# JulHoltzDevelopers/WavesAndEigenvalues.jl

Hardware: AMD Instinct MI355X
Metric: eigenpairs/sec (higher is better)
Workload: dtype f64

## Files before the change

### include/waehip.h

```cpp
#ifndef WAEHIP_H
#define WAEHIP_H
#include <stdint.h>

#ifdef __cplusplus
extern "C" {
#endif

typedef struct wae_family wae_family;

#define WAE_OK                 0
#define WAE_WARN_MAXITER       1
#define WAE_WARN_STAGNATION    2
#define WAE_ERR_INVALID       -1
#define WAE_ERR_BREAKDOWN     -2
#define WAE_ERR_EIGS          -3
#define WAE_ERR_NAN           -4
#define WAE_ERR_HIP           -5

#define WAE_OP_N 0
#define WAE_OP_T 1
#define WAE_OP_C 2

#define WAE_CSC 0
#define WAE_CSR 1
// ... 197 lines not shown
int wae_bench_triad(int32_t device, int64_t n, int32_t reps, double *gbs_out);

int wae_debug_spmv(wae_family *h, int32_t which, int32_t level, int32_t mode, const double *coeffs, int32_t ncoef, const double *X,
                   const double *B, double *Y, double *B2, int32_t r, int32_t op, double jac_w, const uint8_t *cmask, int32_t flags,
                   int64_t *n_in_q, int64_t *n_out_q);

int wae_debug_prolong(wae_family *h, int32_t level, const double *X, const double *B, double *Y, double *norms, int32_t r, const uint8_t *cmask,
                      int32_t flags);

int wae_debug_vcycle(wae_family *h, int32_t level, const double *coeffs, int32_t ncoef, const double *B, double *Y, int32_t r, int32_t op,
                     int32_t flags, const uint8_t *cmask);

enum {
    WAE_VEC_DOTS = 0, WAE_VEC_NORMS, WAE_VEC_DOTS_MULTI, WAE_VEC_AXPY_NEG, WAE_VEC_LINCOMB, WAE_VEC_LINCOMB_ADD, WAE_VEC_AXPY_NEG_NORM,
    WAE_VEC_AXPY_NEG_MULTI, WAE_VEC_DOTS2, WAE_VEC_AXPY2, WAE_VEC_LINCOMB_REP, WAE_VEC_SCALE_INV, WAE_VEC_MASK_COLS, WAE_VEC_EXTRACT_COLS,
    WAE_VEC_BEYN_ACCUM, WAE_VEC_PT_GEMM_BATCH, WAE_VEC_PT_AXPBY_COLS, WAE_VEC_PT_PROJECT, WAE_VEC_DENSE
};
int wae_debug_vec(int32_t device, int32_t op, const int64_t *sz, int32_t nsz, double *const *bufs, const int64_t *lens, int32_t nbuf,
                  const uint8_t *cmask, const int32_t *perm, int32_t *status_out);

enum { WAE_GMRES_INIT = 0, WAE_GMRES_STEP, WAE_GMRES_PAIR, WAE_GMRES_SOLVE_Y };
int wae_debug_gmres(int32_t device, int32_t nb, int32_t m, int32_t histcap, int64_t n, const double *bnorm, const int64_t *ev,
                    const double *evd, int32_t nev, double *pool, int64_t plen, double *cstate, double *dstate, double *snap_relres,
                    int32_t *snap_int, uint8_t *snap_cmask, double *snap_rescale, double *snap_sv, double *snap_vsq);

#ifdef __cplusplus
}
#endif
#endif
```

### wavesandeigenvalues.jl_amd/_lib.py

```python
from __future__ import annotations

import ctypes as C
import os

import numpy as np

_HERE = os.path.dirname(os.path.abspath(__file__))
LIB_PATH = os.environ.get("WAE_LIB_PATH") or os.path.join(_HERE, "csrc", "libwaehip.so")

WAE_OK, WAE_WARN_MAXITER, WAE_WARN_STAGNATION = 0, 1, 2
WAE_ERR_INVALID, WAE_ERR_BREAKDOWN, WAE_ERR_EIGS, WAE_ERR_NAN, WAE_ERR_HIP = -1, -2, -3, -4, -5
OP_N, OP_T, OP_C = 0, 1, 2
CSC, CSR = 0, 1


class SolveInfo(C.Structure):
    _fields_ = [("iters_max", C.c_int32), ("iters_total", C.c_int32), ("n_unconverged", C.c_int32),
                ("levels", C.c_int32), ("relres_max", C.c_double), ("seconds", C.c_double)]

    def as_dict(self):
        return {k: getattr(self, k) for k, _ in self._fields_}


class WaeError(RuntimeError):
# ... 14 lines not shown
    "wae_p1_assemble_cpoint", "wae_p1_assemble_boundary_cpoint", "wae_p2_assemble_cpoint", "wae_p2_assemble_boundary_cpoint",
    "wae_p1_assemble_source", "wae_p1_assemble_source_cpoint", "wae_p2_assemble_source", "wae_p2_assemble_source_cpoint", "wae_forced_response",
    "wae_p2_shape_sensitivity", "wae_p1_shape_sensitivity_cpoint", "wae_p2_shape_sensitivity_cpoint", "wae_p2_shape_sensitivity_flame",
    "wae_bloch_numbering", "wae_bloch_numbering_info", "wae_bloch_numbering_get", "wae_bloch_numbering_free", "wae_bloch_fold",
    "wae_octosplit", "wae_octosplit_info", "wae_octosplit_get", "wae_octosplit_prolong", "wae_octosplit_free",
    "wae_octosplit_prolongator", "wae_solver_setup_nested",
    "wae_octosplit_p2_info", "wae_octosplit_prolongator_p2", "wae_octosplit_prolong_p2", "wae_p2_embedding",
    "wae_locator_create", "wae_locator_info", "wae_locator_find", "wae_locator_set_p2", "wae_locator_weights", "wae_locator_sample",
    "wae_locator_free",
]
BLOCH_IMAGE, BLOCH_AXIS = 1, 2
TALL_MAXCOLS = 64

(VEC_DOTS, VEC_NORMS, VEC_DOTS_MULTI, VEC_AXPY_NEG, VEC_LINCOMB, VEC_LINCOMB_ADD, VEC_AXPY_NEG_NORM, VEC_AXPY_NEG_MULTI, VEC_DOTS2, VEC_AXPY2,
 VEC_LINCOMB_REP, VEC_SCALE_INV, VEC_MASK_COLS, VEC_EXTRACT_COLS, VEC_BEYN_ACCUM, VEC_PT_GEMM_BATCH, VEC_PT_AXPBY_COLS,
 VEC_PT_PROJECT, VEC_DENSE) = range(19)
GMRES_INIT, GMRES_STEP, GMRES_PAIR, GMRES_SOLVE_Y = range(4)


def lib():
    global _lib
    if _lib is not None:
        return _lib
    if not os.path.exists(LIB_PATH):
        raise ImportError(f"{LIB_PATH} not found: build it with `python -c 'import __graft_entry__ as g; g.build()'` "
                          "(hipcc --offload-arch=gfx950). There is no CPU fallback for the product path.")
    L = C.CDLL(LIB_PATH)
    dp = C.POINTER(C.c_double)
    vpp = C.POINTER(C.c_void_p)
    L.wae_last_error.restype = C.c_char_p
    L.wae_version.restype = C.c_char_p
# ... 248 lines not shown
```

### wavesandeigenvalues.jl_amd/csrc/beyn.hip

```cpp
#include <cmath>

#include "solver.h"

static void small_solve(std::vector<zc> &A, std::vector<zc> &b, int n) {
    std::vector<char> dead(n, 0);
    double amax = 0.0;
    for (const zc &a : A) amax = std::max(amax, std::abs(a));
    for (int k = 0; k < n; ++k) {
        int p = k;
        double best = 0.0;
        for (int i = k; i < n; ++i) { const double v = std::abs(A[(size_t)k * n + i]); if (v > best) { best = v; p = i; } }
        if (!(best > 1e-14 * amax)) { dead[k] = 1; continue; }
        if (p != k) {
            for (int j = 0; j < n; ++j) std::swap(A[(size_t)j * n + k], A[(size_t)j * n + p]);
            std::swap(b[k], b[p]);
        }
        const zc inv = 1.0 / A[(size_t)k * n + k];
        for (int i = k + 1; i < n; ++i) {
            const zc f = A[(size_t)k * n + i] * inv;
            if (f == zc(0)) continue;
            for (int j = k + 1; j < n; ++j) A[(size_t)j * n + i] -= f * A[(size_t)j * n + k];
            b[i] -= f * b[k];
        }
    }
// ... 24 lines not shown
    R.wait_w();
    if (R.W.n < R.kact.size() * (size_t)cap * vecl) {
        const size_t need = R.kact.size() * (size_t)cap * vecl;
        const int dev = h->device;
        RbState *Rp = &R;
        R.w_job = std::async(std::launch::async, [Rp, need, dev]() {
            HIP_CHECK(hipSetDevice(dev));
            Rp->W.alloc(need);
        });
    }
    R.Hk.assign(R.kact.size() * (size_t)cap * cap * l, zc(0));
    R.g.assign((size_t)cap * l, zc(0));
    R.Vi.reserve(vecl);
    HIP_CHECK(hipMemcpyAsync(R.Vi.p, Vinter, vecl * sizeof(cplx), hipMemcpyDeviceToDevice, h->stream));
    R.vi_valid = true;
    R.hb.reserve((size_t)4 * (cap + 4) * l); R.alpha.reserve(l); R.alpha2.reserve((size_t)cap * l);
}

static void rb_append_block(wae_family *h, int cnt, const std::vector<std::vector<std::vector<zc>>> &pck) {
    RbState &R = h->rb;
    hipStream_t st = h->stream;
    const int64_t d = h->d;
    const int l = R.l, cap = R.cap, S = R.S;
    const size_t vecl = (size_t)d * l;
    std::vector<cplx> hh((size_t)(S + cnt) * cnt * l), n0((size_t)cnt * l), n1(l);
    const OpDev A0 = h->ops[0].dev(WAE_OP_N);
    cplx *qn = R.Q + (size_t)S * vecl;
    for (int j = 0; j < cnt; ++j) launch_norms(qn + (size_t)j * vecl, d, l, h->partial.p, R.hb.p + (size_t)j * l, st);
    rb_d2h(h, R.hb.p, n0.data(), (size_t)cnt * l);
    static const bool multi_axpy = !(getenv("WAE_RB_MULTI_AXPY") && atoi(getenv("WAE_RB_MULTI_AXPY")) == 0);
    const bool fits = (size_t)S * cnt * l * sizeof(cplx) <= 60 * 1024;
// ... 21 lines not shown
        }
        launch_norms(q, d, l, h->partial.p, R.hb.p, st);
        rb_d2h(h, R.hb.p, n1.data(), l);
        for (int c = 0; c < l; ++c) {
            const double nrm0 = n0[(size_t)j * l + c].x;
            n1[c] = (n1[c].x > 1e-9 * nrm0 && nrm0 > 0.0) ? cplx{n1[c].x, 0.0} : cplx{0.0, 0.0};
        }
        R.alpha.upload(n1.data(), l, st);
        launch_scale_inv(q, R.alpha.p, q, d, l, st);
        HIP_CHECK(hipStreamSynchronize(st));
    }
    launch_dots_multi(qn, vecl, cnt, R.Vi.p, vecl, 1, d, l, h->partial.p, R.hb.p, st);
    rb_d2h(h, R.hb.p, hh.data(), (size_t)cnt * l);
    for (int j = 0; j < cnt; ++j)
        for (int c = 0; c < l; ++c) R.g[(size_t)(S + j) * l + c] = zc(hh[(size_t)j * l + c].x, hh[(size_t)j * l + c].y);
    for (size_t ki = 0; ki < R.kact.size(); ++ki) {
        R.wait_w();
        cplx *Wk = R.W.p + ki * (size_t)cap * vecl;
        cplx *wn = Wk + (size_t)S * vecl;
        upload_pc(h, pck[ki]);
        for (int j = 0; j < cnt; ++j)
            launch_spmv(A0, pc_level(h, 0), l, qn + (size_t)j * vecl, wn + (size_t)j * vecl, nullptr, 0.0, l, MODE_AX, st);
        zc *H = &R.Hk[ki * (size_t)cap * cap * l];
        launch_dots_multi(R.Q, vecl, S + cnt, wn, vecl, cnt, d, l, h->partial.p, R.hb.p, st);
        rb_d2h(h, R.hb.p, hh.data(), (size_t)(S + cnt) * cnt * l);
        for (int i = 0; i < S + cnt; ++i)
            for (int j = 0; j < cnt; ++j)
                for (int c = 0; c < l; ++c) {
                    const cplx v = hh[((size_t)i * cnt + j) * l + c];
                    H[((size_t)(S + j) * cap + i) * l + c] = zc(v.x, v.y);
                }
        zc herm_factor(0);
        bool herm = false;
        {
            static const bool herm_on = !(getenv("WAE_RB_HERMITIAN") && atoi(getenv("WAE_RB_HERMITIAN")) == 0);
            const int kterm = R.kact[ki], pl = h->term_plane[kterm];
            const LevelOp &L0 = h->ops[0];
            for (size_t g = 0; g < L0.groups.size() && herm_on && !herm; ++g)
                for (int q = 0; q < L0.groups[g].nplanes; ++q)
                    if (h->slot_plane[0][(size_t)L0.groups[g].plane0 + q] == pl && L0.groups[g].symmetric && L0.groups[g].is_real) {
// ... 208 lines not shown
            const bool guess = p.guess && R.S > 0;
            const double ta = now_s();
            if (guess) {
                std::vector<cplx> Y;
                if (next_Y.valid()) {
                    Y = next_Y.get();
                    if (p0 + spc < npts) next_Y = launch_coeffs(p0 + spc);
                } else {
                    Y = rb_guess_coeffs(h, p.coeff_table + (size_t)p0 * 2 * T, ns);
                }
                rb_apply_guess(h, Y, ns, h->Xs.p);
            }
            const double tb = now_s();
            h->vc_light = guess && p.light_cycle;
            const int its = solve_chunk(h, bt, pcs, h->Bs.p, h->Xs.p, p.tol, p.maxit, &ci.li, nullptr, guess);
            launch_beyn_accum(h->Xs.p, bt.nb, d, lg, ns, h->zw_dev.p, h->zw_dev.p + ns, npow, Ad, st, p.l_total, p.col0 + cg, h->perm());
            if (rbdbg) HIP_CHECK(hipStreamSynchronize(st));
            const double tc = now_s();
            if (p.keep == BeynPass::raw_to_store) {
                for (int s = 0; s < ns; ++s)
                    launch_extract_cols(h->Xs.p, bt.nb, s * l, l, Q + (size_t)(p.slot0 + p0 + s) * vecl, d, st);
            } else if (p.keep == BeynPass::into_basis || (its > p.enrich_its && R.S + ns <= R.cap)) {
                for (int s = 0; s < ns; ++s)
                    launch_extract_cols(h->Xs.p, bt.nb, s * l, l, Q + (size_t)(R.S + s) * vecl, d, st);
                rb_append(h, ns);
            }
            if (rbdbg) {
                HIP_CHECK(hipStreamSynchronize(st));
                t_guess += tb - ta; t_solve += tc - tb; t_append += now_s() - tc;
            }
        }
// ... 78 lines not shown
```

### wavesandeigenvalues.jl_amd/csrc/debug.hip

```cpp
#include <algorithm>
#include <vector>

#include "solver.h"

namespace {
struct StreamGuard {
    hipStream_t s = nullptr;
    ~StreamGuard() { if (s) (void)hipStreamDestroy(s); }
};
int64_t span(int64_t nv, int64_t stride, int64_t blk) { return nv > 0 ? (nv - 1) * stride + blk : 0; }
void fill_xorshift(std::vector<cplx> &hx) {
    uint64_t s = 0x9E3779B97F4A7C15ull;
    for (auto &v : hx) { s ^= s << 13; s ^= s >> 7; s ^= s << 17; v.x = (double)(s & 0xFFFFF) / 524288.0 - 1.0; v.y = (double)((s >> 20) & 0xFFFFF) / 524288.0 - 1.0; }
}
template <class F> double mean_ms(hipStream_t st, int reps, F &&one) {
    for (int i = 0; i < 3; ++i) one();
    hipEvent_t e0, e1;
    HIP_CHECK(hipEventCreate(&e0));
    HIP_CHECK(hipEventCreate(&e1));
    HIP_CHECK(hipEventRecord(e0, st));
    for (int i = 0; i < reps; ++i) one();
    HIP_CHECK(hipEventRecord(e1, st));
    HIP_CHECK(hipEventSynchronize(e1));
    float ms = 0.f;
// ... 47 lines not shown
            cplx *out = need(2, (int64_t)nv * nb);
            if (scale) launch_dots_scaled(V, (size_t)stride, nv, W, n, (int)nb, want_partial(), out, scale, st, mask());
            else launch_dots(V, (size_t)stride, nv, W, n, (int)nb, want_partial(), out, st, mask());
            break;
        }
        case WAE_VEC_NORMS:
            launch_norms(need(0, blk), n, (int)nb, want_partial(), need(1, nb), st, mask());
            break;
        case WAE_VEC_DOTS_MULTI: {
            const int nv = count_of(2), nw = count_of(3);
            WAE_REQUIRE(nw >= 1 && nw <= 4, "nw in 1..4");
            const cplx *V = need(0, span(nv, S(4), blk)), *W = need(1, span(nw, S(5), blk));
            launch_dots_multi(V, (size_t)S(4), nv, W, (size_t)S(5), nw, n, (int)nb, want_partial(), need(2, (int64_t)nv * nw * nb), st);
            break;
        }
        case WAE_VEC_AXPY_NEG: case WAE_VEC_LINCOMB: case WAE_VEC_LINCOMB_ADD: {
            const int nv = count_of(2);
            const cplx *V = need(0, span(nv, S(3), blk)), *c = need(1, (int64_t)nv * nb);
            cplx *W = need(2, blk);
            if (op == WAE_VEC_AXPY_NEG) launch_axpy_neg(V, (size_t)S(3), nv, c, W, n, (int)nb, st, mask());
            else if (op == WAE_VEC_LINCOMB) launch_lincomb(V, (size_t)S(3), nv, c, W, n, (int)nb, st);
            else launch_lincomb_add(V, (size_t)S(3), nv, c, W, n, (int)nb, st);
            break;
        }
        case WAE_VEC_AXPY_NEG_NORM: {
            const int nv = count_of(2);
            const cplx *V = need(0, span(nv, S(3), blk)), *h = need(1, (int64_t)nv * nb), *base = opt(4, blk);
            cplx *W = need(2, blk), *norms = need(3, nb), *inv = opt(5, nb);
            launch_axpy_neg_norm(V, (size_t)S(3), nv, h, W, n, (int)nb, want_partial(), norms, st, mask(), base, inv);
            break;
// ... 27 lines not shown
            launch_lincomb_rep(need(0, span(nv, S(3), n * l)), (size_t)S(3), nv, need(1, (int64_t)nv * nb), need(2, blk), n, (int)nb, (int)l, st);
            break;
        }
        case WAE_VEC_SCALE_INV:
            launch_scale_inv(need(0, blk), need(1, nb), need(2, blk), n, (int)nb, st, mask());
            break;
        case WAE_VEC_MASK_COLS:
            launch_mask_cols(need(0, blk), need(1, nb), n, (int)nb, st);
            break;
        case WAE_VEC_EXTRACT_COLS: {
            const int64_t off = S(2), l = S(3);
            WAE_REQUIRE(l >= 1 && off + l <= nb, "columns off .. off+l-1 must lie inside the batch");
            launch_extract_cols(need(0, blk), (int)nb, (int)off, (int)l, need(1, n * l), n, st);
            break;
        }
        case WAE_VEC_BEYN_ACCUM: {
            const int64_t l = S(2), nsys = S(3), npow = S(4), lA = S(5) > 0 ? S(5) : l, c0 = S(6);
            WAE_REQUIRE(l >= 1 && nsys >= 1 && nsys * l <= nb && npow >= 1 && npow <= 64 && c0 + l <= lA && lA <= 4096, "bad moment shape");
            if (perm) {
                for (int64_t i = 0; i < n; ++i) WAE_REQUIRE(perm[i] >= 0 && perm[i] < n, "perm entry out of range");
                pm.upload(perm, (size_t)n, st);
            }
            launch_beyn_accum(need(0, blk), (int)nb, n, (int)l, (int)nsys, need(1, nsys), need(2, nsys), (int)npow, need(3, npow * lA * n), st,
                              (int)S(5), (int)c0, perm ? pm.p : nullptr);
            break;
        }
        case WAE_VEC_PT_GEMM_BATCH: {
            const int k = count_of(2), T = count_of(4);
            WAE_REQUIRE(k >= 1 && T >= 1, "k >= 1, T >= 1");
            launch_pt_gemm_batch(need(0, span(k, S(3), blk)), (size_t)S(3), k, need(1, (int64_t)k * T * nb), need(2, blk * T), n, T, (int)nb, st);
            break;
        }
        case WAE_VEC_PT_AXPBY_COLS:
            launch_pt_axpby_cols(need(0, 2 * nb), need(1, blk), need(2, blk), need(3, blk), n, (int)nb, st);
            break;
        case WAE_VEC_PT_PROJECT: {
            const int nd = count_of(2);
            WAE_REQUIRE(nd >= 1, "nd >= 1");
            launch_pt_project(need(0, blk), need(1, blk), need(2, (int64_t)nd * nb), nd, n, (int)nb, st);
// ... 443 lines not shown
```

### wavesandeigenvalues.jl_amd/csrc/family.h

```cpp
#pragma once
#include <algorithm>
#include <chrono>
#include <future>

#include "amg.h"
#include "tiles.h"

struct RbState {
    cplx *Q = nullptr;
    int cap = 0, l = 0, S = 0;
    std::vector<int> kact;
    std::vector<zc> Hk;
    std::vector<zc> g;
    DevBuf<cplx> W, Vi, hb, alpha, alpha2, ycoef;
    std::future<void> w_job;
    void wait_w() { if (w_job.valid()) w_job.get(); }
    bool vi_valid = false;
    ~RbState() { if (w_job.valid()) w_job.wait(); }
};

struct wae_family {
    bool vc_light = false;
    int device = 0;
    hipStream_t stream = nullptr;
    int64_t d = 0;
    int T = 0;
    std::vector<int> term_plane;
    std::vector<zc> term_scale;
    std::vector<int64_t> term_nnz;
    int nplanes = 0;
    std::vector<CsrZ> planes0;
    std::vector<int> perm_h;
    DevBuf<int> perm_dev;
    std::vector<int> tile_row_ptr;
    const int *perm() const { return perm_dev.p; }
    std::vector<LevelOp> ops;
    std::vector<std::vector<int>> slot_plane;
    std::vector<Transfer> xfer;
    int64_t nc = 0;
    DevBuf<cplx> dense_planes, Ainv;
    DevBuf<int> dstatus;
    bool solver_ready = false;
    double jac_w = 0.8;
    double jac_w_post = 0.9;
    double jac_w_light = 0.5;
    int nsweeps = 1, restart = 30, NB = 64;
    std::vector<DevBuf<cplx>> lx, lb, lt;
    DevBuf<cplx> V, W, Z, Xs, Bs, U, partial, hdev, ydev, pcdev, one_dev, io_a, io_b, zw_dev;
    DevBuf<cplx> vsq;
    DevBuf<cplx> rbQ;
// ... 73 lines not shown
```

### wavesandeigenvalues.jl_amd/csrc/setup.hip

```cpp
#include <atomic>
#include <cmath>
#include <exception>
#include <limits>
#include <map>
#include <memory>
#include <tuple>

#include "family.h"

OpDev LevelOp::dev(int op) const {
    OpDev o;
    memset(&o, 0, sizeof(o));
    o.ngroups = (int)groups.size();
    o.nplanes_total = nplanes;
    o.n = n;
    o.diag = diag.p;
    o.conj_diag = (op == WAE_OP_C) ? 1 : 0;
    o.tiles = !tiles.ready ? nullptr : (op == WAE_OP_N || tiles.all_symmetric) ? &tiles.dev : (tiles.ready_t ? &tiles.dev_t : nullptr);
    {
        const LongRows &LR = (op == WAE_OP_N) ? long_n : long_t;
        o.nlong = LR.n;
        o.long_rows = LR.rows.p; o.long_ptr = LR.ptr.p; o.long_col = LR.col.p; o.long_slot = LR.slot.p;
        o.long_val = LR.val.p; o.long_acc = LR.acc.p; o.long_part = LR.part.p;
        o.long_conj = (op == WAE_OP_C) ? 1 : 0;
// ... 608 lines not shown
            h->term_plane[k] = (int)h->planes0.size();
            h->term_scale[k] = 1.0;
            h->planes0.push_back(std::move(A));
        }
    }
    h->nplanes = (int)h->planes0.size();
}
static void renumber_fine_level(wae_family *h, const SetupEnv &env) {
    const double tq0 = now_s();
    TilePlan plan = plan_tiles(union_pattern(h->planes0), 256, env.wcap, TILE_THICK);
    const double tq1 = now_s();
    if (!plan.perm.empty()) {
        host_ranges(h->nplanes, h->nplanes, [&](int64_t q, int64_t, int) { h->planes0[q] = permute_symmetric(h->planes0[q], plan.perm, plan.iperm); });
        h->perm_h = plan.perm;
        h->perm_dev.upload(h->perm_h.data(), h->perm_h.size(), h->stream);
        h->tile_row_ptr = plan.row_ptr;
    }
    if (env.debug)
        fprintf(stderr, "[create] tile plan %.3f s (%zu tiles, largest window %d), permutation of the planes %.3f s\n", tq1 - tq0,
                plan.row_ptr.empty() ? (size_t)0 : plan.row_ptr.size() - 1, plan.wmax, now_s() - tq1);
}

extern "C" int wae_family_create(wae_family **out, int64_t d, int32_t T, int32_t index_bytes, int32_t base, int32_t orientation,
                                 const void *const *ptr, const void *const *idx, const double *const *val, int32_t device) {
    return wae_family_create_opts(out, d, T, index_bytes, base, orientation, ptr, idx, val, device, nullptr, 0);
}

extern "C" int wae_family_create_opts(wae_family **out, int64_t d, int32_t T, int32_t index_bytes, int32_t base, int32_t orientation,
                                      const void *const *ptr, const void *const *idx, const double *const *val, int32_t device,
                                      const double *opts, int32_t nopts) {
// ... 491 lines not shown
```

### wavesandeigenvalues.jl_amd/csrc/vec.hip

```cpp
#include <type_traits>

#include "block_reduce.h"
#include "kernel_helpers.h"

__global__ void fill_zero_kernel(cplx *X, size_t count) {
    for (size_t e = (size_t)blockIdx.x * 256 + threadIdx.x; e < count; e += (size_t)gridDim.x * 256) X[e] = cplx{0.0, 0.0};
}
void launch_fill_zero(cplx *X, size_t count, hipStream_t st) {
    if (!count) return;
    hipLaunchKernelGGL(fill_zero_kernel, dim3(grid_for(count)), dim3(256), 0, st, X, count);
    HIP_CHECK(hipGetLastError());
}
void launch_copy(const cplx *X, cplx *Y, size_t count, hipStream_t st) {
    if (!count) return;
    HIP_CHECK(hipMemcpyAsync(Y, X, count * sizeof(cplx), hipMemcpyDeviceToDevice, st));
}
__global__ void add_kernel(const cplx *__restrict__ X, cplx *__restrict__ Y, size_t count) {
    for (size_t e = (size_t)blockIdx.x * 256 + threadIdx.x; e < count; e += (size_t)gridDim.x * 256) {
        cplx a = X[e], b = Y[e];
        Y[e] = cplx{a.x + b.x, a.y + b.y};
    }
}
void launch_add(const cplx *X, cplx *Y, size_t count, hipStream_t st) {
    if (!count) return;
// ... 138 lines not shown
        }
    }
}
void launch_dots_multi(const cplx *V, size_t sv, int nv, const cplx *W, size_t sw, int nw, int64_t n, int nb, cplx *partial, cplx *out,
                       hipStream_t st) {
    if (nb < 1 || nb > 256 || nw < 1 || nw > 4) throw WaeError(WAE_ERR_INVALID, "dots_multi: nb in 1..256, nw in 1..4");
    int done = 0;
    while (done < nv) {
        const int chunk = std::min(8, nv - done);
        const int nblk = 768;
        hipLaunchKernelGGL((dots_multi_kernel<8, 4>), dim3(nblk), dim3(256), 0, st, V + (size_t)done * sv, sv, chunk, W, sw, nw, n, nb, partial);
        HIP_CHECK(hipGetLastError());
        const int count = chunk * nw * nb;
        launch_reduce_partials(partial, nblk, count, out + (size_t)done * nw * nb, 0, st);
        done += chunk;
    }
}
void launch_dots(const cplx *V, size_t stride, int nv, const cplx *W, int64_t n, int nb, cplx *partial, cplx *out, hipStream_t st,
                 const unsigned char *cmask) {
    dots_impl(V, stride, nv, W, n, nb, partial, out, 0, st, cmask);
}
void launch_dots_scaled(const cplx *V, size_t stride, int nv, const cplx *W, int64_t n, int nb, cplx *partial, cplx *out, const cplx *scale,
                        hipStream_t st, const unsigned char *cmask) {
    dots_impl(V, stride, nv, W, n, nb, partial, out, 0, st, cmask, scale);
}
void launch_norms(const cplx *X, int64_t n, int nb, cplx *partial, cplx *out, hipStream_t st, const unsigned char *cmask) {
    dots_impl(X, 0, 1, X, n, nb, partial, out, 1, st, cmask);
}

constexpr int AXU = 8;
// ... 557 lines not shown
        }
        __syncthreads();
    }
}
void launch_beyn_accum(const cplx *Xi, int nb, int64_t d, int l, int nsys, const cplx *w, const cplx *z, int npow, cplx *A, hipStream_t st,
                       int lA, int c0, const int *perm) {
    if (lA <= 0) lA = l;
    if (!d || nb < 1) return;
    if (nb > 256) throw WaeError(WAE_ERR_INVALID, "beyn_accum: nb must be in 1..256");
    int TR = 2048 / (nb + 1);
    if (TR > 32) TR = 32;
    if (TR < 1) TR = 1;
    const int64_t tiles = (d + TR - 1) / TR;
    const unsigned grid = (unsigned)std::min<int64_t>(tiles, 4096);
    hipLaunchKernelGGL(beyn_accum_kernel, dim3(grid), dim3(256), (size_t)TR * (nb + 1) * sizeof(cplx), st, Xi, nb, d, l, nsys, w, z, npow, A, lA, c0, TR, perm);
    HIP_CHECK(hipGetLastError());
}

__global__ __launch_bounds__(256) void gmres_init_kernel(GmresDev S, const cplx *__restrict__ beta, const unsigned char *__restrict__ done, int use_mask) {
    __shared__ int act[256];
    const int b = threadIdx.x;
    int a = 0;
    if (b < S.nb) {
        S.g[b] = cplx{beta[b].x, 0.0};
        S.sv[b] = 1.0;
        S.vsq[b] = cplx{1.0, 0.0};
        S.conv[b] = done[b] ? 1 : 0;
        S.steps[b] = 0;
        a = done[b] ? 0 : 1;
    }
// ... 322 lines not shown
```

### wavesandeigenvalues.jl_amd/csrc/wae_internal.h

```cpp
#pragma once
#include <hip/hip_runtime.h>
#include <algorithm>
#include <cmath>
#include <complex>
#include <cstdint>
#include <cstdio>
#include <cstring>
#include <stdexcept>
#include <string>
#include <vector>

#include "../../include/waehip.h"

typedef std::complex<double> zc;
typedef double2 cplx;

struct WaeError : std::runtime_error {
    int code;
    WaeError(int c, const std::string &m) : std::runtime_error(m), code(c) {}
};
void wae_set_error(const std::string &m);
int wae_internal_device(const wae_family *h);
hipStream_t wae_internal_stream(const wae_family *h);

// ... 262 lines not shown
void launch_lincomb_add(const cplx *V, size_t stride, int nv, const cplx *y, cplx *X, int64_t n, int nb, hipStream_t s);
void launch_norms(const cplx *X, int64_t n, int nb, cplx *partial, cplx *out, hipStream_t s, const unsigned char *cmask = nullptr);
void launch_scale_inv(const cplx *X, const cplx *alpha, cplx *Y, int64_t n, int nb, hipStream_t s, const unsigned char *cmask = nullptr);
void launch_axpby1(cplx a, const cplx *x, cplx b, const cplx *y, cplx *out, size_t n, hipStream_t s, int conj_x = 0);
void launch_add(const cplx *X, cplx *Y, size_t count, hipStream_t s);
void launch_colmajor_to_inter(const cplx *Xc, int64_t d, int r, cplx *Xi, int nb, hipStream_t s, const int *perm = nullptr);
void launch_inter_to_colmajor(const cplx *Xi, int nb, int64_t d, int r, cplx *Xc, hipStream_t s, const int *perm = nullptr);
void launch_replicate(const cplx *Vc, int64_t d, int l, cplx *Xi, int nb, hipStream_t s, const int *perm = nullptr);
constexpr int PROLONG_NORM_BLOCKS = 1024;
void launch_prolong_add(const int *ptr, const int *col, const double *val, int64_t n, const cplx *Xc, const cplx *X, cplx *Y, int nb, hipStream_t s,
                        const unsigned char *cmask = nullptr, cplx *partial = nullptr, cplx *norms = nullptr);
void launch_reduce_partials(const cplx *partial, int nblk, int count, cplx *out, int do_sqrt, hipStream_t s, const cplx *scale = nullptr,
                            cplx *inv_out = nullptr);
void launch_dots_multi(const cplx *V, size_t sv, int nv, const cplx *W, size_t sw, int nw, int64_t n, int nb, cplx *partial, cplx *out,
                       hipStream_t s);
void launch_gather_rows(const cplx *X, const int *rows, int64_t nrows, int nb, cplx *out, hipStream_t s);
void launch_scatter_add_rows(const cplx *D, const int *rows, int64_t nrows, int nb, cplx *X, hipStream_t s);
void launch_extract_cols(const cplx *X, int nb, int off, int l, cplx *out, int64_t n, hipStream_t s);
void launch_lincomb_rep(const cplx *Q, size_t stride, int nv, const cplx *y, cplx *X, int64_t n, int nb, int l, hipStream_t s);
void launch_mask_cols(cplx *X, const cplx *keep, int64_t n, int nb, hipStream_t s);
void launch_beyn_accum(const cplx *Xi, int nb, int64_t d, int l, int nsys, const cplx *w, const cplx *z, int npow, cplx *A, hipStream_t s,
                       int lA = 0, int c0 = 0, const int *perm = nullptr);
void launch_pt_gemm_batch(const cplx *V, size_t stride, int k, const cplx *G, cplx *U, int64_t d, int T, int nb, hipStream_t s);
void launch_pt_spmv_batch(const OpDev &op, const cplx *pc, const int *plane_col, const cplx *U, int nin, cplx *Y, int nb, int accumulate,
                          hipStream_t s);
void launch_pt_axpby_cols(const cplx *coef, const cplx *x, const cplx *y, cplx *out, int64_t d, int nb, hipStream_t s);
void launch_pt_project(cplx *vk, const cplx *v0, const cplx *dots, int nd, int64_t d, int nb, hipStream_t s);
struct GmresDev {
    int nb, m, histcap;
    cplx *R;
    double *cs;
    cplx *sn;
    cplx *g;
    double *sv;
    cplx *vsq;
    int *conv, *steps, *iters, *histlen, *stalled;
    double *relres, *bnorm;
// ... 20 lines not shown
```

Before: 4.359.

## Batch reduced-basis projections across terms and add row-ordered Beyn accumulation

Adds a dots_terms kernel that computes projections of the basis Q against two term blocks per launch, reusing each loaded basis tile for both terms. All term SpMVs are issued first, then one batched projection and a single device-to-host copy replace the per-term dots_multi launches and copies. Adds a beyn_accum_rows kernel that reads X through the inverse permutation and writes the moment matrix A row-contiguously, aiming for coalesced stores instead of scattered ones. Both paths are on by default behind environment toggles; they add new buffers and shared-memory use, and the dots kernel hardcodes 768 blocks of 512 threads.

Result: no change. 4.396 (median of 6 runs) (+0.8%).

```diff
diff --git a/dev/chunk_boundary_stats.py b/dev/chunk_boundary_stats.py
--- /dev/null
+++ b/dev/chunk_boundary_stats.py
@@ -0,0 +1,62 @@
+#!/usr/bin/env python3
+import csv
+import os
+import re
+import sys
+
+ROOT = os.path.dirname(os.path.dirname(os.path.abspath(__file__)))
+PASSES = 4
+D, L, NS, NPOW = 995328, 8, 8, 4
+
+
+def short(name):
+    return re.sub(r"^void ", "", name.split("(")[0])
+
+
+def load(path):
+    out = {}
+    for r in csv.DictReader(open(path)):
+        k = short(r["Name"])
+        c, t = out.get(k, (0, 0.0))
+        out[k] = (c + int(r["Calls"]), t + float(r["TotalDurationNs"]) / 1e6)
+    return out
+
+
+par, chg = load(sys.argv[1]), load(sys.argv[2])
+par2 = load(sys.argv[3]) if len(sys.argv) > 3 else None
+keys = sorted(set(par) | set(chg), key=lambda k: -max(par.get(k, (0, 0))[1], chg.get(k, (0, 0))[1]))
+dst = os.path.join(ROOT, "profiles", "chunk_boundary_kernel_stats.csv")
+with open(dst, "w", newline="") as f:
+    w = csv.writer(f)
+    head = ["kernel", "parent_calls", "parent_total_ms", "parent_ms_per_pass", "change_calls", "change_total_ms", "change_ms_per_pass",
+            "change_minus_parent_ms_per_pass"]
+    if par2:
+        head.append("second_parent_minus_parent_ms_per_pass")
+    w.writerow(head)
+    for k in keys:
+        pc, pt = par.get(k, (0, 0.0))
+        cc, ct = chg.get(k, (0, 0.0))
+        if max(pt, ct) / PASSES < 0.2:
+            continue
+        row = [k, pc, f"{pt:.2f}", f"{pt / PASSES:.2f}", cc, f"{ct:.2f}", f"{ct / PASSES:.2f}", f"{(ct - pt) / PASSES:.2f}"]
+        if par2:
+            row.append(f"{(par2.get(k, (0, 0.0))[1] - pt) / PASSES:.2f}")
+        w.writerow(row)
+    tp, tc = sum(v[1] for v in par.values()), sum(v[1] for v in chg.values())
+    w.writerow(["all kernels", "", f"{tp:.2f}", f"{tp / PASSES:.2f}", "", f"{tc:.2f}", f"{tc / PASSES:.2f}", f"{(tc - tp) / PASSES:.2f}"]
+               + ([f"{(sum(v[1] for v in par2.values()) - tp) / PASSES:.2f}"] if par2 else []))
+print("wrote", dst)
+
+acc_bytes = 16 * D * L * (NS + 2 * NPOW)
+for side, tab in (("parent", par), ("change", chg)):
+    for k in ("beyn_accum_kernel", "beyn_accum_rows_kernel"):
+        if k in tab:
+            c, t = tab[k]
+            us = 1e3 * t / c
+            print(f"{side:7s} {k:26s} {c:5d} launches  {acc_bytes / 1e9:.3f} GB  {us:7.1f} us  {acc_bytes / us / 1e3:7.1f} GB/s")
+    for k, nw in (("dots_multi_kernel<8, 4>", 4), ("dots_terms_kernel<8, 4>", 8)):
+        if k in tab:
+            c, t = tab[k]
+            us = 1e3 * t / c
+            b = 16 * D * L * (8 + nw)
+            print(f"{side:7s} {k:26s} {c:5d} launches  <= {b / 1e9:.3f} GB  {us:7.1f} us  <= {b / us / 1e3:7.1f} GB/s (mean over all launches)")
diff --git a/include/waehip.h b/include/waehip.h
--- a/include/waehip.h
+++ b/include/waehip.h
@@ -235,7 +235,8 @@
 enum {
     WAE_VEC_DOTS = 0, WAE_VEC_NORMS, WAE_VEC_DOTS_MULTI, WAE_VEC_AXPY_NEG, WAE_VEC_LINCOMB, WAE_VEC_LINCOMB_ADD, WAE_VEC_AXPY_NEG_NORM,
     WAE_VEC_AXPY_NEG_MULTI, WAE_VEC_DOTS2, WAE_VEC_AXPY2, WAE_VEC_LINCOMB_REP, WAE_VEC_SCALE_INV, WAE_VEC_MASK_COLS, WAE_VEC_EXTRACT_COLS,
-    WAE_VEC_BEYN_ACCUM, WAE_VEC_PT_GEMM_BATCH, WAE_VEC_PT_AXPBY_COLS, WAE_VEC_PT_PROJECT, WAE_VEC_DENSE
+    WAE_VEC_BEYN_ACCUM, WAE_VEC_PT_GEMM_BATCH, WAE_VEC_PT_AXPBY_COLS, WAE_VEC_PT_PROJECT, WAE_VEC_DENSE,
+    WAE_VEC_BEYN_ACCUM_ROWS, WAE_VEC_DOTS_TERMS
 };
 int wae_debug_vec(int32_t device, int32_t op, const int64_t *sz, int32_t nsz, double *const *bufs, const int64_t *lens, int32_t nbuf,
                   const uint8_t *cmask, const int32_t *perm, int32_t *status_out);
diff --git a/wavesandeigenvalues.jl_amd/_lib.py b/wavesandeigenvalues.jl_amd/_lib.py
--- a/wavesandeigenvalues.jl_amd/_lib.py
+++ b/wavesandeigenvalues.jl_amd/_lib.py
@@ -52,7 +52,7 @@
 
 (VEC_DOTS, VEC_NORMS, VEC_DOTS_MULTI, VEC_AXPY_NEG, VEC_LINCOMB, VEC_LINCOMB_ADD, VEC_AXPY_NEG_NORM, VEC_AXPY_NEG_MULTI, VEC_DOTS2, VEC_AXPY2,
  VEC_LINCOMB_REP, VEC_SCALE_INV, VEC_MASK_COLS, VEC_EXTRACT_COLS, VEC_BEYN_ACCUM, VEC_PT_GEMM_BATCH, VEC_PT_AXPBY_COLS,
- VEC_PT_PROJECT, VEC_DENSE) = range(19)
+ VEC_PT_PROJECT, VEC_DENSE, VEC_BEYN_ACCUM_ROWS, VEC_DOTS_TERMS) = range(21)
 GMRES_INIT, GMRES_STEP, GMRES_PAIR, GMRES_SOLVE_Y = range(4)
 
 
diff --git a/wavesandeigenvalues.jl_amd/csrc/beyn.hip b/wavesandeigenvalues.jl_amd/csrc/beyn.hip
--- a/wavesandeigenvalues.jl_amd/csrc/beyn.hip
+++ b/wavesandeigenvalues.jl_amd/csrc/beyn.hip
@@ -62,7 +62,8 @@
     R.Vi.reserve(vecl);
     HIP_CHECK(hipMemcpyAsync(R.Vi.p, Vinter, vecl * sizeof(cplx), hipMemcpyDeviceToDevice, h->stream));
     R.vi_valid = true;
-    R.hb.reserve((size_t)4 * (cap + 4) * l); R.alpha.reserve(l); R.alpha2.reserve((size_t)cap * l);
+    R.hb.reserve((size_t)4 * (cap + 4) * l * std::max<size_t>(1, R.kact.size())); R.alpha.reserve(l); R.alpha2.reserve((size_t)cap * l);
+    R.tpart.reserve(DOTS_TERMS_PARTIAL * l);
 }
 
 static void rb_append_block(wae_family *h, int cnt, const std::vector<std::vector<std::vector<zc>>> &pck) {
@@ -114,16 +115,36 @@
     rb_d2h(h, R.hb.p, hh.data(), (size_t)cnt * l);
     for (int j = 0; j < cnt; ++j)
         for (int c = 0; c < l; ++c) R.g[(size_t)(S + j) * l + c] = zc(hh[(size_t)j * l + c].x, hh[(size_t)j * l + c].y);
-    for (size_t ki = 0; ki < R.kact.size(); ++ki) {
+    static const bool terms_fused = !(getenv("WAE_RB_TERMS_FUSED") && atoi(getenv("WAE_RB_TERMS_FUSED")) == 0);
+    const size_t nk = R.kact.size(), hcnt = (size_t)(S + cnt) * cnt * l;
+    std::vector<cplx> hall;
+    if (terms_fused && nk > 1) {
+        R.wait_w();
+        for (size_t ki = 0; ki < nk; ++ki) {
+            cplx *wn = R.W.p + ki * (size_t)cap * vecl + (size_t)S * vecl;
+            upload_pc(h, pck[ki]);
+            for (int j = 0; j < cnt; ++j)
+                launch_spmv(A0, pc_level(h, 0), l, qn + (size_t)j * vecl, wn + (size_t)j * vecl, nullptr, 0.0, l, MODE_AX, st);
+        }
+        R.hb.reserve(nk * hcnt); R.tpart.reserve(DOTS_TERMS_PARTIAL * l);
+        launch_dots_terms(R.Q, vecl, S + cnt, R.W.p + (size_t)S * vecl, vecl, (size_t)cap * vecl, (int)nk, cnt, d, l, R.tpart.p, R.hb.p, hcnt, st);
+        hall.resize(nk * hcnt);
+        rb_d2h(h, R.hb.p, hall.data(), nk * hcnt);
+    }
+    for (size_t ki = 0; ki < nk; ++ki) {
         R.wait_w();
         cplx *Wk = R.W.p + ki * (size_t)cap * vecl;
         cplx *wn = Wk + (size_t)S * vecl;
-        upload_pc(h, pck[ki]);
-        for (int j = 0; j < cnt; ++j)
-            launch_spmv(A0, pc_level(h, 0), l, qn + (size_t)j * vecl, wn + (size_t)j * vecl, nullptr, 0.0, l, MODE_AX, st);
         zc *H = &R.Hk[ki * (size_t)cap * cap * l];
-        launch_dots_multi(R.Q, vecl, S + cnt, wn, vecl, cnt, d, l, h->partial.p, R.hb.p, st);
-        rb_d2h(h, R.hb.p, hh.data(), (size_t)(S + cnt) * cnt * l);
+        if (hall.empty()) {
+            upload_pc(h, pck[ki]);
+            for (int j = 0; j < cnt; ++j)
+                launch_spmv(A0, pc_level(h, 0), l, qn + (size_t)j * vecl, wn + (size_t)j * vecl, nullptr, 0.0, l, MODE_AX, st);
+            launch_dots_multi(R.Q, vecl, S + cnt, wn, vecl, cnt, d, l, h->partial.p, R.hb.p, st);
+            rb_d2h(h, R.hb.p, hh.data(), hcnt);
+        } else {
+            std::copy(hall.begin() + ki * hcnt, hall.begin() + (ki + 1) * hcnt, hh.begin());
+        }
         for (int i = 0; i < S + cnt; ++i)
             for (int j = 0; j < cnt; ++j)
                 for (int c = 0; c < l; ++c) {
@@ -362,7 +383,11 @@
             const double tb = now_s();
             h->vc_light = guess && p.light_cycle;
             const int its = solve_chunk(h, bt, pcs, h->Bs.p, h->Xs.p, p.tol, p.maxit, &ci.li, nullptr, guess);
-            launch_beyn_accum(h->Xs.p, bt.nb, d, lg, ns, h->zw_dev.p, h->zw_dev.p + ns, npow, Ad, st, p.l_total, p.col0 + cg, h->perm());
+            static const bool accum_rows = !(getenv("WAE_ACCUM_ROWS") && atoi(getenv("WAE_ACCUM_ROWS")) == 0);
+            if (accum_rows && (!h->perm() || h->iperm()))
+                launch_beyn_accum_rows(h->Xs.p, bt.nb, d, lg, ns, h->zw_dev.p, h->zw_dev.p + ns, npow, Ad, st, p.l_total, p.col0 + cg, h->iperm());
+            else
+                launch_beyn_accum(h->Xs.p, bt.nb, d, lg, ns, h->zw_dev.p, h->zw_dev.p + ns, npow, Ad, st, p.l_total, p.col0 + cg, h->perm());
             if (rbdbg) HIP_CHECK(hipStreamSynchronize(st));
             const double tc = now_s();
             if (p.keep == BeynPass::raw_to_store) {
diff --git a/wavesandeigenvalues.jl_amd/csrc/debug.hip b/wavesandeigenvalues.jl_amd/csrc/debug.hip
--- a/wavesandeigenvalues.jl_amd/csrc/debug.hip
+++ b/wavesandeigenvalues.jl_amd/csrc/debug.hip
@@ -85,6 +85,15 @@
             launch_dots_multi(V, (size_t)S(4), nv, W, (size_t)S(5), nw, n, (int)nb, want_partial(), need(2, (int64_t)nv * nw * nb), st);
             break;
         }
+        case WAE_VEC_DOTS_TERMS: {
+            const int nv = count_of(2), nw = count_of(3), nt = count_of(6);
+            WAE_REQUIRE(nw >= 1 && nw <= 4 && nt >= 1, "nw in 1..4, nt >= 1");
+            const cplx *V = need(0, span(nv, S(4), blk)), *W = need(1, span(nt, S(7), span(nw, S(5), blk)));
+            partial.alloc(DOTS_TERMS_PARTIAL * (size_t)nb);
+            launch_dots_terms(V, (size_t)S(4), nv, W, (size_t)S(5), (size_t)S(7), nt, nw, n, (int)nb, partial.p, need(2, (int64_t)nt * nv * nw * nb),
+                              (size_t)nv * nw * nb, st);
+            break;
+        }
         case WAE_VEC_AXPY_NEG: case WAE_VEC_LINCOMB: case WAE_VEC_LINCOMB_ADD: {
             const int nv = count_of(2);
             const cplx *V = need(0, span(nv, S(3), blk)), *c = need(1, (int64_t)nv * nb);
@@ -142,15 +151,27 @@
             launch_extract_cols(need(0, blk), (int)nb, (int)off, (int)l, need(1, n * l), n, st);
             break;
         }
-        case WAE_VEC_BEYN_ACCUM: {
+        case WAE_VEC_BEYN_ACCUM: case WAE_VEC_BEYN_ACCUM_ROWS: {
             const int64_t l = S(2), nsys = S(3), npow = S(4), lA = S(5) > 0 ? S(5) : l, c0 = S(6);
             WAE_REQUIRE(l >= 1 && nsys >= 1 && nsys * l <= nb && npow >= 1 && npow <= 64 && c0 + l <= lA && lA <= 4096, "bad moment shape");
             if (perm) {
                 for (int64_t i = 0; i < n; ++i) WAE_REQUIRE(perm[i] >= 0 && perm[i] < n, "perm entry out of range");
-                pm.upload(perm, (size_t)n, st);
+                if (op == WAE_VEC_BEYN_ACCUM_ROWS) {
+                    std::vector<int> inv((size_t)n, -1);
+                    for (int64_t i = 0; i < n; ++i) inv[(size_t)perm[i]] = (int)i;
+                    for (int64_t i = 0; i < n; ++i) WAE_REQUIRE(inv[(size_t)i] >= 0, "perm is not a permutation");
+                    pm.upload(inv.data(), (size_t)n, st);
+                    HIP_CHECK(hipStreamSynchronize(st));
+                } else {
+                    pm.upload(perm, (size_t)n, st);
+                }
             }
-            launch_beyn_accum(need(0, blk), (int)nb, n, (int)l, (int)nsys, need(1, nsys), need(2, nsys), (int)npow, need(3, npow * lA * n), st,
-                              (int)S(5), (int)c0, perm ? pm.p : nullptr);
+            if (op == WAE_VEC_BEYN_ACCUM_ROWS)
+                launch_beyn_accum_rows(need(0, blk), (int)nb, n, (int)l, (int)nsys, need(1, nsys), need(2, nsys), (int)npow, need(3, npow * lA * n), st,
+                                       (int)S(5), (int)c0, perm ? pm.p : nullptr);
+            else
+                launch_beyn_accum(need(0, blk), (int)nb, n, (int)l, (int)nsys, need(1, nsys), need(2, nsys), (int)npow, need(3, npow * lA * n), st,
+                                  (int)S(5), (int)c0, perm ? pm.p : nullptr);
             break;
         }
         case WAE_VEC_PT_GEMM_BATCH: {
diff --git a/wavesandeigenvalues.jl_amd/csrc/family.h b/wavesandeigenvalues.jl_amd/csrc/family.h
--- a/wavesandeigenvalues.jl_amd/csrc/family.h
+++ b/wavesandeigenvalues.jl_amd/csrc/family.h
@@ -13,6 +13,7 @@
     std::vector<zc> Hk;
     std::vector<zc> g;
     DevBuf<cplx> W, Vi, hb, alpha, alpha2, ycoef;
+    DevBuf<cplx> tpart;
     std::future<void> w_job;
     void wait_w() { if (w_job.valid()) w_job.get(); }
     bool vi_valid = false;
@@ -34,6 +35,8 @@
     DevBuf<int> perm_dev;
     std::vector<int> tile_row_ptr;
     const int *perm() const { return perm_dev.p; }
+    DevBuf<int> iperm_dev;
+    const int *iperm() const { return iperm_dev.p; }
     std::vector<LevelOp> ops;
     std::vector<std::vector<int>> slot_plane;
     std::vector<Transfer> xfer;
diff --git a/wavesandeigenvalues.jl_amd/csrc/setup.hip b/wavesandeigenvalues.jl_amd/csrc/setup.hip
--- a/wavesandeigenvalues.jl_amd/csrc/setup.hip
+++ b/wavesandeigenvalues.jl_amd/csrc/setup.hip
@@ -646,6 +646,7 @@
         host_ranges(h->nplanes, h->nplanes, [&](int64_t q, int64_t, int) { h->planes0[q] = permute_symmetric(h->planes0[q], plan.perm, plan.iperm); });
         h->perm_h = plan.perm;
         h->perm_dev.upload(h->perm_h.data(), h->perm_h.size(), h->stream);
+        h->iperm_dev.upload(plan.iperm.data(), plan.iperm.size(), h->stream);
         h->tile_row_ptr = plan.row_ptr;
     }
     if (env.debug)
diff --git a/wavesandeigenvalues.jl_amd/csrc/vec.hip b/wavesandeigenvalues.jl_amd/csrc/vec.hip
--- a/wavesandeigenvalues.jl_amd/csrc/vec.hip
+++ b/wavesandeigenvalues.jl_amd/csrc/vec.hip
@@ -176,6 +176,94 @@
         const int count = chunk * nw * nb;
         launch_reduce_partials(partial, nblk, count, out + (size_t)done * nw * nb, 0, st);
         done += chunk;
+    }
+}
+template <int MAXV, int NW>
+__global__ __launch_bounds__(512) void dots_terms_kernel(const cplx *__restrict__ V, size_t sv, int nv, const cplx *__restrict__ W, size_t sw, size_t st,
+                                                         int nw, int64_t n, int nb, cplx *__restrict__ partial) {
+    static_assert(MAXV % 2 == 0, "each group loads half of the tile");
+    __shared__ cplx vt[MAXV][256];
+    __shared__ cplx sm2[2][256];
+    const int g = threadIdx.x >> 8, tid = threadIdx.x & 255;
+    const int R = 256 / nb;
+    const int b = tid % nb, rl = tid / nb;
+    const cplx *__restrict__ Wg = W + (size_t)g * st;
+    cplx acc[MAXV][NW];
+#pragma unroll
+    for (int i = 0; i < MAXV; ++i)
+#pragma unroll
+        for (int j = 0; j < NW; ++j) acc[i][j] = cplx{0.0, 0.0};
+    const int64_t step = (int64_t)gridDim.x * R;
+    cplx wn[NW], vn[MAXV / 2];
+    auto fetch = [&](int64_t row0) {
+        const int64_t row = (rl < R && row0 + rl < n) ? row0 + rl : row0;
+        const size_t e = (size_t)row * nb + b;
+#pragma unroll
+        for (int j = 0; j < NW; ++j) wn[j] = j < nw ? Wg[(size_t)j * sw + e] : cplx{0.0, 0.0};
+#pragma unroll
+        for (int k = 0; k < MAXV / 2; ++k) vn[k] = 2 * k + g < nv ? V[(size_t)(2 * k + g) * sv + e] : cplx{0.0, 0.0};
+    };
+    int64_t row0 = (int64_t)blockIdx.x * R;
+    if (row0 < n) fetch(row0);
+    for (; row0 < n; row0 += step) {
+        cplx w[NW];
+#pragma unroll
+        for (int j = 0; j < NW; ++j) w[j] = wn[j];
+#pragma unroll
+        for (int k = 0; k < MAXV / 2; ++k) vt[2 * k + g][tid] = vn[k];
+        const bool live = rl < R && row0 + rl < n;
+        if (row0 + step < n) fetch(row0 + step);
+        __syncthreads();
+        if (live) {
+#pragma unroll
+            for (int i = 0; i < MAXV; ++i) {
+                if (i < nv) {
+                    const cplx v = vt[i][tid];
+#pragma unroll
+                    for (int j = 0; j < NW; ++j) {
+                        acc[i][j].x += v.x * w[j].x + v.y * w[j].y;
+                        acc[i][j].y += v.x * w[j].y - v.y * w[j].x;
+                    }
+                }
+            }
+        }
+        __syncthreads();
+    }
+    cplx *sm = sm2[g];
+    cplx *pg = partial + (size_t)g * gridDim.x * nv * nw * nb;
+#pragma unroll
+    for (int i = 0; i < MAXV; ++i) {
+#pragma unroll
+        for (int j = 0; j < NW; ++j) {
+            if (i < nv && j < nw) {
+                sm[tid] = acc[i][j];
+                __syncthreads();
+                if (tid < nb) {
+                    cplx s = sm[tid];
+                    for (int k = 1; k < R; ++k) s = vadd(s, sm[k * nb + tid]);
+                    pg[((size_t)blockIdx.x * nv * nw + (size_t)i * nw + j) * nb + tid] = s;
+                }
+                __syncthreads();
+            }
+        }
+    }
+}
+void launch_dots_terms(const cplx *V, size_t sv, int nv, const cplx *W, size_t sw, size_t st, int nt, int nw, int64_t n, int nb, cplx *partial,
+                       cplx *out, size_t so, hipStream_t stream) {
+    if (nb < 1 || nb > 256 || nw < 1 || nw > 4 || nt < 1) throw WaeError(WAE_ERR_INVALID, "dots_terms: nb in 1..256, nw in 1..4, nt >= 1");
+    for (int t0 = 0; t0 < nt; t0 += 2) {
+        const cplx *Wt = W + (size_t)t0 * st;
+        cplx *ot = out + (size_t)t0 * so;
+        if (t0 + 1 == nt) { launch_dots_multi(V, sv, nv, Wt, sw, nw, n, nb, partial, ot, stream); break; }
+        for (int done = 0; done < nv; done += 8) {
+            const int chunk = std::min(8, nv - done);
+            const int nblk = 768;
+            hipLaunchKernelGGL((dots_terms_kernel<8, 4>), dim3(nblk), dim3(512), 0, stream, V + (size_t)done * sv, sv, chunk, Wt, sw, st, nw, n, nb, partial);
+            HIP_CHECK(hipGetLastError());
+            const int count = chunk * nw * nb;
+            for (int g = 0; g < 2; ++g)
+                launch_reduce_partials(partial + (size_t)g * nblk * count, nblk, count, ot + (size_t)g * so + (size_t)done * nw * nb, 0, stream);
+        }
     }
 }
 void launch_dots(const cplx *V, size_t stride, int nv, const cplx *W, int64_t n, int nb, cplx *partial, cplx *out, hipStream_t st,
@@ -763,6 +851,63 @@
     const int64_t tiles = (d + TR - 1) / TR;
     const unsigned grid = (unsigned)std::min<int64_t>(tiles, 4096);
     hipLaunchKernelGGL(beyn_accum_kernel, dim3(grid), dim3(256), (size_t)TR * (nb + 1) * sizeof(cplx), st, Xi, nb, d, l, nsys, w, z, npow, A, lA, c0, TR, perm);
+    HIP_CHECK(hipGetLastError());
+}
+__global__ __launch_bounds__(256) void beyn_accum_rows_kernel(const cplx *__restrict__ Xi, int nb, int64_t d, int l, int nsys,
+                                                              const cplx *__restrict__ w, const cplx *__restrict__ z, int npow, cplx *__restrict__ A,
+                                                              int lA, int c0, int TR, const int *__restrict__ iperm) {
+    extern __shared__ cplx tile[];
+    const int ld = nb + 1;
+    const int tid = threadIdx.x;
+    for (int64_t row0 = (int64_t)blockIdx.x * TR; row0 < d; row0 += (int64_t)gridDim.x * TR) {
+        for (int e = tid; e < TR * nb; e += 256) {
+            const int r = e / nb, col = e - r * nb;
+            const int64_t row = row0 + r;
+            tile[r * ld + col] = (row < d) ? Xi[(size_t)(iperm ? (int64_t)iperm[row] : row) * nb + col] : cplx{0.0, 0.0};
+        }
+        __syncthreads();
+        for (int idx = tid; idx < TR * l; idx += 256) {
+            const int c = idx / TR, r = idx - c * TR;
+            const int64_t row = row0 + r;
+            if (row >= d) continue;
+            for (int p0 = 0; p0 < npow; p0 += ACC_MAXP) {
+                const int np = npow - p0 < ACC_MAXP ? npow - p0 : ACC_MAXP;
+                cplx acc[ACC_MAXP];
+#pragma unroll
+                for (int p = 0; p < ACC_MAXP; ++p) acc[p] = cplx{0.0, 0.0};
+                for (int s = 0; s < nsys; ++s) {
+                    cplx t = cmul(w[s], tile[r * ld + s * l + c]);
+                    const cplx zs = z[s];
+                    for (int q = 0; q < p0; ++q) t = cmul(t, zs);
+#pragma unroll
+                    for (int p = 0; p < ACC_MAXP; ++p) {
+                        if (p < np) { acc[p].x += t.x; acc[p].y += t.y; t = cmul(t, zs); }
+                    }
+                }
+#pragma unroll
+                for (int p = 0; p < ACC_MAXP; ++p) {
+                    if (p < np) {
+                        cplx *dst = A + ((size_t)(p0 + p) * lA + c0 + c) * d + row;
+                        const cplx a = *dst;
+                        *dst = cplx{a.x + acc[p].x, a.y + acc[p].y};
+                    }
+                }
+            }
+        }
+        __syncthreads();
+    }
+}
+void launch_beyn_accum_rows(const cplx *Xi, int nb, int64_t d, int l, int nsys, const cplx *w, const cplx *z, int npow, cplx *A, hipStream_t st,
+                            int lA, int c0, const int *iperm) {
+    if (lA <= 0) lA = l;
+    if (!d || nb < 1) return;
+    if (nb > 256) throw WaeError(WAE_ERR_INVALID, "beyn_accum: nb must be in 1..256");
+    int TR = 32;
+    while (TR > 1 && (size_t)TR * (nb + 1) * sizeof(cplx) > 40 * 1024) TR >>= 1;
+    const int64_t tiles = (d + TR - 1) / TR;
+    const unsigned grid = (unsigned)std::min<int64_t>(tiles, 4096);
+    hipLaunchKernelGGL(beyn_accum_rows_kernel, dim3(grid), dim3(256), (size_t)TR * (nb + 1) * sizeof(cplx), st, Xi, nb, d, l, nsys, w, z, npow, A, lA, c0, TR,
+                       iperm);
     HIP_CHECK(hipGetLastError());
 }
 
diff --git a/wavesandeigenvalues.jl_amd/csrc/wae_internal.h b/wavesandeigenvalues.jl_amd/csrc/wae_internal.h
--- a/wavesandeigenvalues.jl_amd/csrc/wae_internal.h
+++ b/wavesandeigenvalues.jl_amd/csrc/wae_internal.h
@@ -300,6 +300,9 @@
                             cplx *inv_out = nullptr);
 void launch_dots_multi(const cplx *V, size_t sv, int nv, const cplx *W, size_t sw, int nw, int64_t n, int nb, cplx *partial, cplx *out,
                        hipStream_t s);
+constexpr size_t DOTS_TERMS_PARTIAL = (size_t)2 * 768 * 32;
+void launch_dots_terms(const cplx *V, size_t sv, int nv, const cplx *W, size_t sw, size_t st, int nt, int nw, int64_t n, int nb, cplx *partial,
+                       cplx *out, size_t so, hipStream_t s);
 void launch_gather_rows(const cplx *X, const int *rows, int64_t nrows, int nb, cplx *out, hipStream_t s);
 void launch_scatter_add_rows(const cplx *D, const int *rows, int64_t nrows, int nb, cplx *X, hipStream_t s);
 void launch_extract_cols(const cplx *X, int nb, int off, int l, cplx *out, int64_t n, hipStream_t s);
@@ -307,6 +310,8 @@
 void launch_mask_cols(cplx *X, const cplx *keep, int64_t n, int nb, hipStream_t s);
 void launch_beyn_accum(const cplx *Xi, int nb, int64_t d, int l, int nsys, const cplx *w, const cplx *z, int npow, cplx *A, hipStream_t s,
                        int lA = 0, int c0 = 0, const int *perm = nullptr);
+void launch_beyn_accum_rows(const cplx *Xi, int nb, int64_t d, int l, int nsys, const cplx *w, const cplx *z, int npow, cplx *A, hipStream_t s,
+                            int lA = 0, int c0 = 0, const int *iperm = nullptr);
 void launch_pt_gemm_batch(const cplx *V, size_t stride, int k, const cplx *G, cplx *U, int64_t d, int T, int nb, hipStream_t s);
 void launch_pt_spmv_batch(const OpDev &op, const cplx *pc, const int *plane_col, const cplx *U, int nin, cplx *Y, int nb, int accumulate,
                           hipStream_t s);
```
